# liuq-lab/bayesgm

Hardware: AMD Instinct MI355X
Metric: posterior samples/sec (whole node), CausalBGM N=1e6 p=200 (higher is better)
Workload: dtype f32

## Files before the change

### bayesgm_amd/csrc/bgm_host.h

```cpp
#pragma once
#include <hip/hip_runtime.h>

#include <algorithm>
#include <string>
#include <vector>

#include "../../include/bgm_hip.h"
#include "causal_kernels.h"
#include "fit_types.h"

void bgm_set_error(const std::string &msg);

#define BGM_HIP_CHECK(expr)                                                                  \
  do {                                                                                       \
    hipError_t _e = (expr);                                                                  \
    if (_e != hipSuccess) {                                                                  \
      bgm_set_error(std::string(#expr) + ": " + hipGetErrorString(_e));                      \
      return BGM_E_HIP;                                                                      \
    }                                                                                        \
  } while (0)

template <class T>
static int bgm_reserve(T *&ptr, size_t &cap, size_t count) {
  if (cap >= count) return BGM_OK;
// ... 44 lines not shown
};

struct bgm_handle {
  int device = 0;
  int n_cus = 256;
  int disc_norm = 0;
  bool configured = false;
  bgm_causal_config cfg{};
  int q = 0, p = 0;
  HostNet nets[4];
  CausalMeta meta{};
  int KT1 = 0, KSL1 = 0, NTL = 0;
  float *blob_dev = nullptr;
  size_t blob_cap = 0;
  bool blob_valid = false;
  float *sblob_dev = nullptr;
  size_t sblob_cap = 0;
  bool sblob_valid = false;
  float *gblob_dev = nullptr, *gram_w_dev = nullptr, *uc_dev = nullptr;
  size_t gblob_cap = 0, gram_w_cap = 0, uc_cap = 0;
  bool gram_valid = false;
  bool mh_direct = false;
  bool mh_all_ksteps = false;
  CausalMeta gmeta{};
  int precision = 0;
  unsigned char *bx_blob_dev = nullptr;
  size_t bx_cap = 0;
  float *eff_cache = nullptr;
  size_t eff_cache_cap = 0;
  int outcome_cache = 2;
  unsigned long long *eff_stats_dev = nullptr;
  unsigned long long eff_total = 0;
  unsigned long long ev_total = 0;
  float *ev_z = nullptr; unsigned *ev_meta = nullptr; int *ev_tile = nullptr, *ev_slot_cnt = nullptr; float *ev_out = nullptr, *ev_carry = nullptr;
  size_t ev_z_cap = 0, ev_meta_cap = 0, ev_tile_cap = 0, ev_slot_cap = 0, ev_out_cap = 0, ev_carry_cap = 0;
  int ev_carry_flip = 0;
  long long ev_budget_bytes = 0;
  int ev_fallbacks = 0;
  bool bx_valid = false;
  alignas(8) unsigned char bx_meta_store[192];
  const int32_t *prior_seg = nullptr;
  const float *prior_tab = nullptr;
  int prior_segments = 0;
  float *ra_scale = nullptr;
  const float *ra_up = nullptr, *ra_dn = nullptr;
  int ra_n = 0;
// ... 128 lines not shown
```

### bayesgm_amd/csrc/causal_api.hip

```cpp
#include <algorithm>
#include <string>
#include <vector>
#include <cstdio>
#include <cmath>
#include <cstring>
#include <cstdlib>

#include "causal_launch.h"
#include "bnf_det_host.h"
#include "gx_host.h"

static thread_local std::string g_err;
void bgm_set_error(const std::string &msg) { g_err = msg; }

extern "C" const char *bgm_last_error(void) { return g_err.c_str(); }
extern "C" const char *bgm_version(void) { return "bayesgm_amd-hip 0.1 (gfx950)"; }

extern "C" int bgm_create(bgm_handle **out, int device) {
  if (!out) { bgm_set_error("bgm_create: out == NULL"); return BGM_E_INVALID; }
  BGM_HIP_CHECK(hipSetDevice(device));
  hipDeviceProp_t prop;
  BGM_HIP_CHECK(hipGetDeviceProperties(&prop, device));
  if (std::string(prop.gcnArchName).find("gfx950") == std::string::npos) {
    bgm_set_error(std::string("bgm_create: device is ") + prop.gcnArchName + ", this library is built for gfx950 only");
    return BGM_E_UNSUPPORTED;
  }
  bgm_handle *h = new bgm_handle();
  h->device = device;
  h->n_cus = prop.multiProcessorCount;
  const char *direct = std::getenv("BGM_MH_DIRECT_LIKELIHOOD");
  h->mh_direct = direct != nullptr && std::strcmp(direct, "0") != 0;
  const char *all_ks = std::getenv("BGM_MH_ALL_KSTEPS");
  h->mh_all_ksteps = all_ks != nullptr && std::strcmp(all_ks, "0") != 0;
  *out = h;
  return BGM_OK;
}

extern "C" int bgm_set_disc_norm(bgm_handle *h, int32_t mode) {
  if (!h || (mode != 0 && mode != 1)) { bgm_set_error("bgm_set_disc_norm: mode must be 0 (batch statistics) or 1 (inference mode)"); return BGM_E_INVALID; }
  h->disc_norm = mode;
  return BGM_OK;
}

extern "C" int bgm_destroy(bgm_handle *h) {
  if (!h) return BGM_OK;
  hipSetDevice(h->device);
  if (h->blob_dev) hipFree(h->blob_dev);
  if (h->eblob_dev) hipFree(h->eblob_dev);
  if (h->sblob_dev) hipFree(h->sblob_dev);
  if (h->gblob_dev) hipFree(h->gblob_dev);
  if (h->gram_w_dev) hipFree(h->gram_w_dev);
  if (h->uc_dev) hipFree(h->uc_dev);
  if (h->bx_blob_dev) hipFree(h->bx_blob_dev);
  if (h->acc_scratch) hipFree(h->acc_scratch);
  if (h->eff_cache) hipFree(h->eff_cache);
  if (h->eff_stats_dev) hipFree(h->eff_stats_dev);
// ... 126 lines not shown
  const int q1 = q + 1;
  int KT1, KSL1, NTL;
  if (!bgm_causal_shape(q1, p + 1, KT1, KSL1, NTL)) {
    bgm_set_error("no compiled kernel shape contains this model (needs sum(z_dims) <= 19 and v_dim <= 207, or <= 159 when sum(z_dims) > 11)");
    return BGM_E_UNSUPPORTED;
  }
  h->KT1 = KT1; h->KSL1 = KSL1; h->NTL = NTL;
  CausalMeta &m = h->meta;
  std::memset(&m, 0, sizeof(m));
  m.q = q; m.p = p; m.binary = h->cfg.binary_treatment ? 1 : 0;
  m.sig_pc = p % 16; m.sig_slot = bgm_sig_slot(p, NTL);
  auto s2 = [](float s) { return s > 0.0f ? s * s : -1.0f; };
  m.sig2_v = s2(h->cfg.sigma_v); m.sig2_x = s2(h->cfg.sigma_x); m.sig2_y = s2(h->cfg.sigma_y);
  m.n_gh = h->cfg.n_hidden_g - 1;
  int off = 0;
  auto take = [&](int n) { int o = off; off += (n + 3) / 4 * 4; return o; };
  m.w1g = take(16 * KT1 * 64); m.w1f = take(16 * KT1 * 64); m.w1h = take(16 * KT1 * 64);
  m.b1g = take(64); m.b1f = take(64); m.b1h = take(64);
  m.wg = take(m.n_gh * 4096); m.bg = take(m.n_gh * 64);
  m.wgl = take(64 * 16 * NTL); m.bgl = take(16 * NTL);
  m.wf2 = take(64 * 32); m.bf2 = take(32); m.wf3 = take(32 * 16); m.bf3 = take(16); m.wf4 = take(16 * 16); m.bf4 = take(16);
  m.wh2 = take(64 * 32); m.bh2 = take(32); m.wh3 = take(32 * 16); m.bh3 = take(16); m.wh4 = take(16 * 16); m.bh4 = take(16);
  m.wxf = take(64);
  m.total = off;
  if ((size_t)m.total * 4 > 160 * 1024) {
    bgm_set_error("model does not fit the 160 KiB LDS-resident layout (" + std::to_string(m.total * 4) + " B); p <= 207 with default widths");
    return BGM_E_UNSUPPORTED;
  }
  blob.assign(m.total, 0.0f);
  auto ident = [](int rho) { return rho; };
  const L1RowMaps rm(h);
  pack_layer(blob, m.w1g, G.W(0), q, 64, KT1, 4, [&](int rho) { return rm.g(rho); });
  pack_layer(blob, m.w1f, F.W(0), z0 + z1 + 1, 64, KT1, 4, [&](int rho) { return rm.f(rho); });
  pack_layer(blob, m.w1h, H.W(0), z0 + z2, 64, KT1, 4, [&](int rho) { return rm.h(rho); });
  causal_l1_masks(h, KT1, KSL1, m.l1f, m.l1h, m.l1b);
  pack_bias(blob, m.b1g, G.b(0), 64, 4); pack_bias(blob, m.b1f, F.b(0), 64, 4); pack_bias(blob, m.b1h, H.b(0), 64, 4);
  for (int l = 0; l < m.n_gh; ++l) {
    pack_layer(blob, m.wg + l * 4096, G.W(1 + l), 64, 64, 4, 4, ident);
    pack_bias(blob, m.bg + l * 64, G.b(1 + l), 64, 4);
  }
  const int LG = (int)G.dims.size() - 2;
  {
    std::vector<float> Wp, bp;
    bgm_g_last_padded(G.W(LG), G.b(LG), p, NTL, Wp, bp);
    pack_layer(blob, m.wgl, Wp.data(), 64, 16 * NTL, 4, NTL, ident);
    pack_bias(blob, m.bgl, bp.data(), 16 * NTL, NTL);
  }
  pack_layer(blob, m.wf2, F.W(1), 64, 32, 4, 2, ident); pack_bias(blob, m.bf2, F.b(1), 32, 2);
  pack_layer(blob, m.wf3, F.W(2), 32, 8, 2, 1, ident); pack_bias(blob, m.bf3, F.b(2), 8, 1);
// ... 13 lines not shown
  const int w3[2] = {m.wf3, m.wh3}, b3[2] = {m.bf3, m.bh3}, w4[2] = {m.wf4, m.wh4}, b4[2] = {m.bf4, m.bh4};
#pragma unroll
  for (int k = 0; k < 2; ++k) {
    if (in(w3[k], 32 * 16)) {
      const int rho = (i - w3[k]) >> 4, f = tail_pos_to_feature((i - w3[k]) & 15);
      dst[i] = f >= 0 ? src[w3[k] + rho * 16 + f] * BGM_LRS_W : 0.0f;
      return;
    }
    if (in(b3[k], 16)) {
      const int f = tail_pos_to_feature(i - b3[k]);
      dst[i] = f >= 0 ? src[b3[k] + f] : 0.0f;
      return;
    }
    if (in(w4[k], 16 * 16)) {
      const int f = tail_pos_to_feature((i - w4[k]) >> 4), c = (i - w4[k]) & 3;
      dst[i] = (f >= 0 && c < 2) ? src[w4[k] + f * 16 + c] * BGM_LRS_W : 0.0f;
      return;
    }
    if (in(b4[k], 16)) {
      const int c = (i - b4[k]) & 3;
      dst[i] = c < 2 ? src[b4[k] + c] : 0.0f;
      return;
    }
  }
  const bool scaled = in(m.wg, m.n_gh * 4096) || in(m.wgl, 64 * 16 * NTL) || in(m.wf2, 64 * 32) || in(m.wh2, 64 * 32);
  dst[i] = scaled ? src[i] * BGM_LRS_W : src[i];
}

int bgm_causal_sampling_blob(bgm_handle *h, hipStream_t stream) {
  if (!h->blob_valid) h->sblob_valid = false;
  int rc = bgm_causal_build_blob(h, stream);
  if (rc) return rc;
  if (h->sblob_valid) return BGM_OK;
  const size_t n = (size_t)h->meta.total;
  if ((rc = bgm_reserve(h->sblob_dev, h->sblob_cap, n))) return rc;
  h->gram_valid = false;
  hipLaunchKernelGGL(causal_scale_blob_kernel, dim3((unsigned)((n + 255) / 256)), dim3(256), 0, stream, h->blob_dev, h->sblob_dev,
                     h->meta, h->NTL);
  BGM_HIP_CHECK(hipGetLastError());
  h->sblob_valid = true;
  return BGM_OK;
}

static bool gram_wanted(const bgm_handle *h, int NTL) { return !h->mh_direct && h->precision == 0 && NTL > 2; }

static float packed_w(const std::vector<float> &b, int off, int NT, int i, int o) {
// ... 21 lines not shown
    }
    act.swap(nxt);
  }
  std::vector<float> a0(64), W((size_t)64 * p), wt((size_t)65 * p), G(64 * 64);
  for (int i = 0; i < 64; ++i) a0[i] = (float)act[i];
  for (int i = 0; i < 64; ++i)
    for (int c = 0; c < p; ++c) W[(size_t)i * p + c] = packed_w(sb, m.wgl, NTL, i, c);
  for (int c = 0; c < p; ++c) {
    double s = sb[m.bgl + c];
    for (int i = 0; i < 64; ++i) { s += (double)W[(size_t)i * p + c] * (double)a0[i]; wt[(size_t)c * 64 + i] = W[(size_t)i * p + c]; }
    wt[(size_t)64 * p + c] = (float)s;
  }
  for (int i = 0; i < 64; ++i)
    for (int k = 0; k <= i; ++k) {
      double s = 0.0;
      for (int c = 0; c < p; ++c) s += (double)W[(size_t)i * p + c] * (double)W[(size_t)k * p + c];
      G[i * 64 + k] = G[k * 64 + i] = (float)s;
    }
  CausalMeta gm = m;
  gm.bgl = m.wgl + 4096;
  const int shift = (gm.bgl + 132) - m.wf2;
  for (int CausalMeta::*f : {&CausalMeta::wf2, &CausalMeta::bf2, &CausalMeta::wf3, &CausalMeta::bf3, &CausalMeta::wf4, &CausalMeta::bf4,
                             &CausalMeta::wh2, &CausalMeta::bh2, &CausalMeta::wh3, &CausalMeta::bh3, &CausalMeta::wh4, &CausalMeta::bh4,
                             &CausalMeta::wxf, &CausalMeta::total})
    gm.*f += shift;
  std::vector<float> gb((size_t)gm.total, 0.0f);
  std::copy(sb.begin(), sb.begin() + m.wgl, gb.begin());
  pack_layer(gb, gm.wgl, G.data(), 64, 64, 4, 4, [](int rho) { return rho; });
  for (int i = 0; i < 64; ++i) { gb[gm.bgl + i] = a0[i]; gb[gm.bgl + 64 + i] = packed_w(sb, m.wgl, NTL, i, m.sig_slot); }
  gb[gm.bgl + 128] = sb[m.bgl + m.sig_slot];
  std::copy(sb.begin() + m.wf2, sb.end(), gb.begin() + gm.wf2);
  if (int rc = bgm_reserve(h->gblob_dev, h->gblob_cap, gb.size())) return rc;
  if (int rc = bgm_reserve(h->gram_w_dev, h->gram_w_cap, wt.size())) return rc;
  BGM_HIP_CHECK(hipMemcpyAsync(h->gblob_dev, gb.data(), gb.size() * sizeof(float), hipMemcpyHostToDevice, stream));
  BGM_HIP_CHECK(hipMemcpyAsync(h->gram_w_dev, wt.data(), wt.size() * sizeof(float), hipMemcpyHostToDevice, stream));
  BGM_HIP_CHECK(hipStreamSynchronize(stream));
  h->gmeta = gm;
  h->gram_valid = true;
  h->hmc_valid = false;
  return BGM_OK;
}

static __global__ __launch_bounds__(256) void causal_gram_prepass_kernel(const float *wt, const float *v, long long n, int p, float *uc) {
  extern __shared__ __attribute__((aligned(16))) float sw[];
  for (int i = threadIdx.x; i < 65 * p; i += blockDim.x) sw[i] = wt[i];
  __syncthreads();
  const long long row = (long long)blockIdx.x * blockDim.x + threadIdx.x;
// ... 72 lines not shown
  if (gx_wanted(h)) {
    return gx_logpost(h, x, y, v, z, n, out, stream);
  }
  if (bnf_det_wanted(h)) {
    if (h->prior_seg || h->precision != 0) { bgm_set_error("bgm_causal_logpost: the conditional prior / split precision exist for the LDS-resident shapes only"); return BGM_E_UNSUPPORTED; }
    return bnf_det_logpost(h, x, y, v, z, n, out, stream);
  }
  int rc = bgm_causal_sampling_blob(h, stream);
  if (rc) return rc;
  const int grid = mh_grid(h, n);
  if (h->precision != 0) return bgm_causal_bx3_logpost(h, x, y, v, z, n, out, grid, stream);
  if (h->prior_seg) return bgm_causal_prior_logpost(h, x, y, v, z, n, out, grid, stream);
  return bgm_causal_dispatch(h, "kernel", [&](auto s) {
    using S = decltype(s);
    return bgm_launch(causal_logpost_kernel<S::KT1, S::KSL1, S::NTL, MH_R, MH_WAVES>, grid, MH_WAVES, h->meta.total * 4, stream,
                      h->sblob_dev, h->meta, x, y, v, z, n, out, nullptr, nullptr);
  });
}

template <int EFFECT>
static int launch_mh(bgm_handle *h, const CausalMhKArgs &ka, int grid, int lds, hipStream_t stream) {
  return bgm_causal_dispatch(h, "MH kernel", [&](auto s) {
    using S = decltype(s);
    return bgm_launch(ka.uc ? causal_mh_kernel<S::KT1, S::KSL1, S::NTL, MH_R, MH_WAVES, EFFECT, 0, (S::NTL > 2)>
                            : causal_mh_kernel<S::KT1, S::KSL1, S::NTL, MH_R, MH_WAVES, EFFECT>,
                      grid, MH_WAVES, lds, stream, ka);
  });
}

extern "C" int bgm_causal_mh_run(bgm_handle *h, const bgm_mh_args *a, void *stream_) {
  if (!h || !h->configured) { bgm_set_error("bgm_causal_mh_run: handle not configured"); return BGM_E_STATE; }
  if (!a) { bgm_set_error("bgm_causal_mh_run: NULL args"); return BGM_E_INVALID; }
  if (a->n <= 0 || a->n_iters <= 0) return BGM_OK;
  if (!a->x_dev || !a->y_dev || !a->v_dev || !a->state_dev || !a->logp_dev) { bgm_set_error("bgm_causal_mh_run: NULL data pointer"); return BGM_E_INVALID; }
  if (a->row_base + a->n > 0xFFFFFFFFll) { bgm_set_error("bgm_causal_mh_run: row index exceeds the 32-bit RNG counter"); return BGM_E_INVALID; }
  if (a->effect == BGM_EFFECT_ADRF && (!a->x_values_dev || a->n_doses <= 0 || !a->adrf_partial_dev)) { bgm_set_error("bgm_causal_mh_run: ADRF effect needs x_values / adrf_partial"); return BGM_E_INVALID; }
  if (a->effect == BGM_EFFECT_ITE && !a->ite_dev) { bgm_set_error("bgm_causal_mh_run: ITE effect needs ite_dev"); return BGM_E_INVALID; }
  if (a->effect == BGM_EFFECT_ADRF && h->cfg.binary_treatment) { bgm_set_error("bgm_causal_mh_run: ADRF effect on a binary-treatment model"); return BGM_E_INVALID; }
  const int it_end = a->it_begin + a->n_iters;
  if ((a->effect != BGM_EFFECT_NONE || a->draws_dev) && it_end - a->burn_in > a->n_keep) { bgm_set_error("bgm_causal_mh_run: iterations beyond burn_in + n_keep"); return BGM_E_INVALID; }
  hipStream_t stream = (hipStream_t)stream_;
  BGM_HIP_CHECK(hipSetDevice(h->device));
  if (h->ra_scale) {
    const char *path = gx_wanted(h) ? "the general-width engine (hidden widths outside the compiled families)"
                       : bnf_det_wanted(h) ? "the streamed-fragment kernels (no LDS-resident compiled shape holds the model)"
                       : h->precision != 0 ? "the split-precision kernels (bgm_causal_set_precision)"
                       : h->prior_seg ? "the conditional latent prior (bgm_causal_set_prior)" : nullptr;
    if (path) { bgm_set_error(std::string("bgm_causal_mh_run: the per-chain proposal scale (bgm_causal_set_row_scale) does not exist for ") + path); return BGM_E_UNSUPPORTED; }
  }
// ... 271 lines not shown
```

### bayesgm_amd/csrc/causal_event_api.hip

```cpp
#include <algorithm>
#include <cstdlib>
#include <string>

#include "causal_launch.h"
#include "causal_event_kernels.h"

static constexpr int EV_SPREAD_WAVES = 4, EV_SPREAD_LDS_FLOATS = 8192;

bool bgm_causal_event_wanted(const bgm_handle *h, int effect, int n_doses) {
  static const bool off = std::getenv("BGM_NO_EVENT_SPLIT") != nullptr;
  if (off || h->outcome_cache != 2) return false;
  if (effect == BGM_EFFECT_ITE) return h->cfg.binary_treatment != 0;
  return effect == BGM_EFFECT_ADRF && n_doses >= 1 && (n_doses + 3) / 4 <= EV_NCMAX;
}

template <class T>
static int ev_try_reserve(T *&ptr, size_t &cap, size_t need) {
  if (cap >= need) return BGM_OK;
  if (ptr) BGM_HIP_CHECK(hipFree(ptr));
  ptr = nullptr; cap = 0;
  if (hipMalloc((void **)&ptr, need * sizeof(T)) != hipSuccess) {
    (void)hipGetLastError();
    ptr = nullptr;
    return 1;
// ... 46 lines not shown
  h->ev_z_cap = h->ev_meta_cap = h->ev_tile_cap = h->ev_slot_cap = h->ev_out_cap = h->ev_carry_cap = 0;
}

int bgm_causal_event_mh_launch(bgm_handle *h, CausalMhKArgs &ka, int grid, int lds, hipStream_t stream) {
  ka.ev_z = h->ev_z; ka.ev_meta = h->ev_meta; ka.tile_ev = h->ev_tile; ka.slot_cnt = h->ev_slot_cnt;
  if (h->precision != 0) return bgm_causal_bx3_mh_launch(h, ka, 3, grid, stream);
  if (h->prior_seg) return bgm_causal_prior_mh_launch(h, ka, 3, grid, lds, stream);
  if (ka.row_scale) return bgm_causal_rowadapt_mh_launch(h, ka, 3, grid, lds, stream);
  return bgm_causal_dispatch(h, "event-form MH kernel", [&](auto s) {
    using S = decltype(s);
    return bgm_launch(ka.uc ? causal_mh_kernel<S::KT1, S::KSL1, S::NTL, MH_R, MH_WAVES, 3, 0, (S::NTL > 2)>
                            : causal_mh_kernel<S::KT1, S::KSL1, S::NTL, MH_R, MH_WAVES, 3>,
                      grid, MH_WAVES, lds, stream, ka);
  });
}

int bgm_causal_event_finish(bgm_handle *h, const CausalMhKArgs &ka, int grid, int first, hipStream_t stream, int effect) {
  CausalEventFArgs fa{};
  fa.blob = ka.blob; fa.ev_z = h->ev_z; fa.slot_cnt = h->ev_slot_cnt; fa.ev_cap = ka.ev_cap; fa.n_doses = ka.n_doses;
  fa.x_values = ka.x_values; fa.ev_out = reinterpret_cast<float2 *>(h->ev_out); fa.eff_stats = ka.eff_stats; fa.m = ka.m;
  constexpr int FW = 4, WPS = 2;
  const int rc = bgm_causal_dispatch(h, "event-form outcome-net kernel", [&](auto s) {
    using S = decltype(s);
    const int lds = 4 * (16 * S::KT1 * 64 + 64 + 64 * 32 + 32 + 32 * 16 + 16 + 16 * 16 + 16 + 64);
    return bgm_launch(effect == BGM_EFFECT_ITE ? causal_event_f_ite_kernel<S::KT1, S::KSL1, FW, WPS>
                                               : causal_event_f_kernel<S::KT1, S::KSL1, FW, WPS>,
                      grid * MH_WAVES * WPS / FW, FW, lds, stream, fa);
  });
  if (rc) return rc;
  if (effect == BGM_EFFECT_ITE) {
    CausalEventIteArgs ia{};
    ia.n = ka.n; ia.row_base = ka.row_base; ia.it_begin = ka.it_begin; ia.n_iters = ka.n_iters; ia.burn_in = ka.burn_in; ia.n_keep = ka.n_keep;
    ia.sample_y = ka.sample_y; ia.n_slots = grid * MH_WAVES; ia.k0 = ka.k0; ia.k1 = ka.k1;
    ia.ev_meta = h->ev_meta; ia.tile_ev = h->ev_tile; ia.ev_cap = ka.ev_cap; ia.ev_out = reinterpret_cast<const float4 *>(h->ev_out);
    const size_t carry_floats = (size_t)((ka.n + 15) / 16) * 64 * 2;
    h->ev_carry_flip = first ? 0 : (h->ev_carry_flip ^ 1);
    ia.carry_in = reinterpret_cast<const float4 *>(h->ev_carry + (h->ev_carry_flip ^ 1) * carry_floats);
    ia.carry_out = reinterpret_cast<float4 *>(h->ev_carry + h->ev_carry_flip * carry_floats);
    ia.first = first; ia.ite = ka.ite;
    hipLaunchKernelGGL(causal_event_ite_kernel, dim3((unsigned)((ka.n + 255) / 256)), dim3(256), 0, stream, ia);
    BGM_HIP_CHECK(hipGetLastError());
    return BGM_OK;
  }
  CausalEventSpreadArgs sa{};
  sa.n = ka.n; sa.row_base = ka.row_base; sa.it_begin = ka.it_begin; sa.n_iters = ka.n_iters; sa.burn_in = ka.burn_in; sa.n_keep = ka.n_keep;
  sa.sample_y = ka.sample_y; sa.n_doses = ka.n_doses; sa.k0 = ka.k0; sa.k1 = ka.k1;
  sa.ev_meta = h->ev_meta; sa.tile_ev = h->ev_tile; sa.ev_cap = ka.ev_cap; sa.ev_out = reinterpret_cast<const float2 *>(h->ev_out);
  const size_t carry_floats = (size_t)((ka.n + 15) / 16) * (size_t)((ka.n_doses + 3) / 4) * 64 * 2;
  h->ev_carry_flip = first ? 0 : (h->ev_carry_flip ^ 1);
// ... 15 lines not shown
```

### bayesgm_amd/csrc/causal_event_kernels.h

```cpp
#pragma once
#include "causal_kernels.h"

#define EV_NCMAX 8

struct CausalEventFArgs {
  const float *blob;
  const float *ev_z;
  const int *slot_cnt;
  long long ev_cap;
  int n_doses;
  const float *x_values;
  float2 *ev_out;
  unsigned long long *eff_stats;
  CausalMeta m;
};

template <int KT1, int KSL1, int WAVES, int WPS>
__global__ __launch_bounds__(64 * WAVES) void causal_event_f_kernel(CausalEventFArgs a) {
  extern __shared__ __attribute__((aligned(16))) float lds[];
  CausalMeta m = a.m;
  {
    int off = 0;
    auto put = [&](int src, int nfl) {
      for (int i = threadIdx.x; i < nfl; i += 64 * WAVES) lds[off + i] = a.blob[src + i];
      const int o = off;
      off += nfl;
      return o;
    };
    m.w1f = put(a.m.w1f, 16 * KT1 * 64); m.b1f = put(a.m.b1f, 64);
    m.wf2 = put(a.m.wf2, 64 * 32); m.bf2 = put(a.m.bf2, 32); m.wf3 = put(a.m.wf3, 32 * 16); m.bf3 = put(a.m.bf3, 16);
    m.wf4 = put(a.m.wf4, 16 * 16); m.bf4 = put(a.m.bf4, 16); m.wxf = put(a.m.wxf, 64);
    __syncthreads();
  }
  const int lane = threadIdx.x & 63, wave = threadIdx.x >> 6;
  const int j = lane & 15, g = lane >> 4, lane_off = 64 * g + j;
  const long long wid = (long long)blockIdx.x * WAVES + wave;
  const long long slot = wid / WPS;
  const int sub = (int)(wid % WPS);
  const int cnt = a.slot_cnt[slot];
  const int n_calls = (a.n_doses + 3) >> 2;
  if (a.eff_stats != nullptr && lane == 0 && sub == 0 && cnt > 0) atomicAdd(&a.eff_stats[1], (unsigned long long)cnt);
  for (int e0 = 16 * sub; e0 < cnt; e0 += 16 * WPS) {
    BGM_NO_HOIST();
    const int el = (e0 + j < cnt) ? e0 + j : cnt - 1;
    const float *zr = a.ev_z + (slot * a.ev_cap + el) * (long long)m.q;
    f32x4 zs[1][KT1];
#pragma unroll
    for (int t = 0; t < KT1; ++t)
#pragma unroll
      for (int r = 0; r < 4; ++r) {
        const int f = 16 * t + 4 * r + g;
        zs[0][t][r] = (f < m.q) ? zr[f] : 0.0f;
      }
    const unsigned rowid[1] = {0u};
    const bool valid[1] = {true};
    float2 *out = a.ev_out + ((slot * a.ev_cap + e0) >> 4) * (long long)n_calls * 64;
    causal_effects<KT1, KSL1, 1, 1, true, true, true>(lds, m, lane_off, g, j, lane, zs, rowid, valid, 0ll, 16ll, 0u, 0ll, 1, 0, a.n_doses,
                                                      a.x_values, nullptr, nullptr, 0u, 0u, out);
  }
}

template <int KT1, int KSL1, int WAVES, int WPS>
__global__ __launch_bounds__(64 * WAVES) void causal_event_f_ite_kernel(CausalEventFArgs a) {
  extern __shared__ __attribute__((aligned(16))) float lds[];
  CausalMeta m = a.m;
  {
    int off = 0;
    auto put = [&](int src, int nfl) {
      for (int i = threadIdx.x; i < nfl; i += 64 * WAVES) lds[off + i] = a.blob[src + i];
      const int o = off;
      off += nfl;
      return o;
    };
    m.w1f = put(a.m.w1f, 16 * KT1 * 64); m.b1f = put(a.m.b1f, 64);
    m.wf2 = put(a.m.wf2, 64 * 32); m.bf2 = put(a.m.bf2, 32); m.wf3 = put(a.m.wf3, 32 * 16); m.bf3 = put(a.m.bf3, 16);
    m.wf4 = put(a.m.wf4, 16 * 16); m.bf4 = put(a.m.bf4, 16); m.wxf = put(a.m.wxf, 64);
    __syncthreads();
  }
  const int lane = threadIdx.x & 63, wave = threadIdx.x >> 6;
  const int j = lane & 15, g = lane >> 4, lane_off = 64 * g + j;
  const long long wid = (long long)blockIdx.x * WAVES + wave;
// ... 183 lines not shown
```

### bayesgm_amd/csrc/causal_kernels.h

```cpp
#pragma once
#include "bgm_device.h"
#include "row_tails.h"

struct CausalMeta {
  int q, p;
  int sig_pc, sig_slot;
  int binary;
  float sig2_v, sig2_x, sig2_y;
  int n_gh;
  int w1g, w1f, w1h, b1g, b1f, b1h;
  int wg, bg;
  int wgl, bgl;
  int wf2, bf2, wf3, bf3, wf4, bf4;
  int wh2, bh2, wh3, bh3, wh4, bh4;
  int wxf;
  int total;
  unsigned l1f, l1h, l1b;
};
__host__ __device__ constexpr bool causal_l1_masked(int KT1, int PRIOR) { return !(PRIOR != 0 && KT1 > 1); }

struct CausalMhKArgs {
  const float *blob;
  const float *x, *y, *v;
  const float *uc;
  long long n, row_base;
  float *state, *logp;
  int init, it_begin, n_iters, burn_in;
  float q_sd;
  unsigned k0, k1;
  unsigned *acc_count;
  float *draws;
  int n_keep, sample_y, n_doses;
  const float *x_values;
  float *adrf_partial;
  float *ite;
  unsigned long long *clk;
  const int *seg;
  const float *prior_tab;
  float *eff_cache;
  int eff_skip;
  unsigned long long *eff_stats;
  float *ev_z;
// ... 425 lines not shown
    unsigned long long tsec[8] = {0, 0, 0, 0, 0, 0, 0, 0}, tlast = 0;
    causal_logp<KT1, KSL1, NTL, R>(lds, m, lane_off, g, j, zin, vreg, xr, yr, lp, tsec, tlast);
#else
    causal_logp<KT1, KSL1, NTL, R>(lds, m, lane_off, g, j, zin, vreg, xr, yr, lp);
#endif
    if constexpr (PRIOR) {
      PriorRow<KT1> pr;
      const long long rowc = (row0 + j < n) ? row0 + j : n - 1;
      pr.load(seg, prior_tab, rowc, m.q, g);
      lp[0] += pr.correction(zin[0], m.q, g);
    }
#pragma unroll
    for (int rr = 0; rr < R; ++rr) {
      const long long row = row0 + 16 * rr + j;
      if (g == 0 && row < n) out[row] = lp[rr];
    }
  }
}

__device__ __forceinline__ float pick_by_group(int g, float v0, float v1, float v2, float v3) {
  return g == 0 ? v0 : (g == 1 ? v1 : (g == 2 ? v2 : v3));
}

template <int KT1, int KSL1, int R, int EFFECT, bool GROUPING = true, bool CACHE = false, bool EVAL_ONLY = false, bool L1MASK = true,
          bool ROWS = false, bool TAILS = false>
__device__ __forceinline__ void causal_effects(const float *lds, const CausalMeta &m, int lane_off, int g, int j,
                                               int lane, const f32x4 (&zs)[R][KT1], const unsigned (&rowid)[R],
                                               const bool (&valid)[R], long long row0, long long n, unsigned it,
                                               long long d, int n_keep, int sample_y, int n_doses,
                                               const float *x_values, float *adrf_slot, float *ite, unsigned k0,
                                               unsigned k1, float2 *cache = nullptr, float *ite_c = nullptr,
                                               float *row_mom = nullptr, float *row_y = nullptr, int label = 0,
                                               float *row_tails = nullptr, int k_tail = 0) {
  static_assert(!ROWS || (EFFECT == 1 && R == 1 && GROUPING && !CACHE && !EVAL_ONLY), "ROWS: the grouped finish of the dose-response sums");
  static_assert(EFFECT != 4 || (R == 1 && !CACHE && !EVAL_ONLY && !ROWS), "EFFECT 4: the label sums of one row tile per wave");
  static_assert(!TAILS || ROWS, "TAILS: the tail buffers of the per-row dose-response");
  constexpr bool ARMS = (EFFECT == 2 || EFFECT == 4);
  BGM_NO_HOIST();
  f32x4 z0in[R][KT1];
#pragma unroll
  for (int rr = 0; rr < R; ++rr)
#pragma unroll
    for (int t = 0; t < KT1; ++t)
#pragma unroll
      for (int r = 0; r < 4; ++r) z0in[rr][t][r] = (16 * t + 4 * r + g == m.q) ? 0.0f : zs[rr][t][r];
  f32x4 base[R][4];
  if constexpr (L1MASK) dense_masked<KT1, KSL1, 4, R>(lds + m.w1f, lds + m.b1f, lane_off, g, z0in, base, m.l1b);
  else dense<KT1, KSL1, 4, R>(lds + m.w1f, lds + m.b1f, lane_off, g, z0in, base);
  f32x4 wx[4];
#pragma unroll
  for (int t = 0; t < 4; ++t) wx[t] = *reinterpret_cast<const f32x4 *>(lds + m.wxf + 16 * t + 4 * g);
  const int nd = ARMS ? (CACHE && n_doses == 0 ? 0 : 2) : n_doses;
  constexpr int DB = ARMS ? 2 : 4;
  constexpr bool GROUPED = (EFFECT == 1 && R == 1 && GROUPING);
  const int n_calls = (nd + 3) >> 2, n_own = GROUPED ? (n_calls & ~3) : 0;
  f32x4 nz[R];
#pragma unroll
  for (int rr = 0; rr < R; ++rr) nz[rr] = f32x4{0.0f, 0.0f, 0.0f, 0.0f};
  for (int kb = 0; kb < n_calls; ++kb) {
    BGM_NO_HOIST();
    const bool own = kb < n_own;
    const int c4 = kb & ~3, p4 = kb & 3;
    if (!EVAL_ONLY && sample_y && (!own || p4 == 0)) {
#pragma unroll
      for (int rr = 0; rr < R; ++rr) nz[rr] = box_muller4(philox4x32_10(rowid[rr], it, (unsigned)(own ? c4 + g : kb), TAG_YNOISE, k0, k1));
    }
    float xk[DB];
#pragma unroll
    for (int e = 0; e < DB; ++e) {
      const int k = own ? 4 * (c4 + e) + p4 : 4 * kb + e;
      xk[e] = ARMS ? (e == 0 ? 1.0f : 0.0f) : x_values[k < nd ? k : nd - 1];
    }
    float mu[DB * R], sr[DB * R];
#ifndef BGM_NO_JIT_EFFECTS
    if constexpr (R == 1) {
      f32x4 a2[DB][2];
#pragma unroll
// ... 170 lines not shown
  if (g == 0 && row < n) ite[row * (long long)n_keep + d] = y1 - y0;
}

template <int KT1>
__device__ __forceinline__ void causal_event_append(const CausalMhKArgs &a, int q, long long slot, int &ev_cnt, bool ev, int g, int j,
                                                    const f32x4 (&z)[KT1], int it) {
  const unsigned m16 = (unsigned)(__ballot(ev && g == 0) & 0xFFFFull);
  if (m16 == 0u) return;
  if (ev) {
    const long long e = slot * a.ev_cap + ev_cnt + __popc(m16 & ((1u << j) - 1u));
    float *ez = a.ev_z + e * (long long)q;
#pragma unroll
    for (int t = 0; t < KT1; ++t)
#pragma unroll
      for (int r = 0; r < 4; ++r) {
        const int f = 16 * t + 4 * r + g;
        if (f < q) ez[f] = z[t][r];
      }
    if (g == 0) a.ev_meta[e] = ((unsigned)(it - a.it_begin) << 4) | (unsigned)j;
  }
  ev_cnt += __popc(m16);
}

template <int KT1, int KSL1, int NTL, int R, int WAVES, int EFFECT, int PRIOR = 0, bool GRAM = false, bool ROWADAPT = false>
__global__ __launch_bounds__(64 * WAVES) void causal_mh_kernel(CausalMhKArgs a) {
  static_assert(PRIOR == 0 || R == 1, "conditional prior: one row tile per wave");
  constexpr bool L1M = causal_l1_masked(KT1, PRIOR);
  extern __shared__ __attribute__((aligned(16))) float lds[];
  const CausalMeta &m = a.m;
  lds_fill(lds, a.blob, m.total);
  const int lane = threadIdx.x & 63, wave = threadIdx.x >> 6;
  const int j = lane & 15, g = lane >> 4, lane_off = 64 * g + j;
  const long long n = a.n;
  const long long n_tiles = (n + 16 * R - 1) / (16 * R);
  const long long slot = (long long)blockIdx.x * WAVES + wave;
  const long long n_slots = (long long)gridDim.x * WAVES;
  const unsigned long long clk_c0 = __builtin_readcyclecounter(), clk_r0 = __builtin_amdgcn_s_memrealtime();
#ifdef BGM_PROF
  unsigned long long tsec[8] = {0, 0, 0, 0, 0, 0, 0, 0}, tlast = 0;
#endif
  const int wave_u = __builtin_amdgcn_readfirstlane(wave);
  volatile __attribute__((address_space(3))) int *prog =
      (volatile __attribute__((address_space(3))) int *)((__attribute__((address_space(3))) float *)lds + m.total);
  if (lane == 0) prog[wave_u] = 0;
  int tiles_done = 0;
  [[maybe_unused]] int ev_cnt = 0;

  for (long long tile = slot; tile < n_tiles; tile += n_slots) {
    const long long row0 = tile * 16 * R;
// ... 126 lines not shown
        if (a.draws != nullptr) {
#pragma unroll
          for (int rr = 0; rr < R; ++rr) {
            const long long row = row0 + 16 * rr + j;
            if (row < n) {
              float *dr = a.draws + (d * n + row) * (long long)m.q;
#pragma unroll
              for (int t = 0; t < KT1; ++t)
#pragma unroll
                for (int r = 0; r < 4; ++r) {
                  const int f = 16 * t + 4 * r + g;
                  if (f < m.q) dr[f] = zs[rr][t][r];
                }
            }
          }
        }
        if constexpr (EFFECT == 3) {
          static_assert(R == 1, "event mode: one row tile per wave");
          causal_event_append<KT1>(a, m.q, slot, ev_cnt, valid[0] && (moved[0] || (a.ev_first && it == a.it_begin)), g, j, zs[0], it);
        } else if constexpr (EFFECT == 1 && R == 1) {
          float2 *cache = reinterpret_cast<float2 *>(a.eff_cache) + slot * (long long)((a.n_doses + 3) >> 2) * 64;
          float *adrf_slot = a.adrf_partial + slot * (long long)a.n_doses * a.n_keep;
          const bool skip = a.eff_skip && eff_cached && accmask == 0ull;
          causal_effects<KT1, KSL1, R, EFFECT, true, true, false, L1M>(lds, m, lane_off, g, j, lane, zs, rowid, valid, row0, n, (unsigned)it, d, a.n_keep,
                                                            a.sample_y, skip ? 0 : a.n_doses, a.x_values, adrf_slot, a.ite, a.k0, a.k1, cache);
          if (skip) causal_effects_cached(g, j, lane, rowid[0], valid[0], (unsigned)it, d, a.sample_y, a.n_doses, adrf_slot, a.k0, a.k1, cache);
          eff_cached = true;
          n_eff_skipped += skip ? 1u : 0u;
        } else if constexpr (EFFECT == 2 && R == 1) {
          const bool skip = a.eff_skip && eff_cached && accmask == 0ull;
          causal_effects<KT1, KSL1, R, EFFECT, true, true, false, L1M>(lds, m, lane_off, g, j, lane, zs, rowid, valid, row0, n, (unsigned)it, d, a.n_keep,
                                                            a.sample_y, skip ? 0 : 2, a.x_values, a.adrf_partial, a.ite, a.k0, a.k1, nullptr, ite_c);
          if (skip) causal_ite_cached(g, j, rowid[0], row0 + j, n, (unsigned)it, d, a.n_keep, a.sample_y, a.ite, a.k0, a.k1, ite_c);
          eff_cached = true;
          n_eff_skipped += skip ? 1u : 0u;
        } else if constexpr (EFFECT != 0) {
          causal_effects<KT1, KSL1, R, EFFECT, true, false, false, L1M>(lds, m, lane_off, g, j, lane, zs, rowid, valid, row0, n, (unsigned)it, d,
                                                a.n_keep, a.sample_y, a.n_doses, a.x_values,
                                                a.adrf_partial + slot * (long long)((EFFECT == 2) ? 2 : a.n_doses) * a.n_keep,
                                                a.ite, a.k0, a.k1);
        }
      }
    }
    if constexpr (EFFECT != 0 && R == 1) {
      if (a.eff_stats != nullptr && lane == 0 && n_eff_skipped != 0u) atomicAdd(&a.eff_stats[0], (unsigned long long)n_eff_skipped);
    }
    if constexpr (EFFECT == 3) {
// ... 171 lines not shown
```

### bayesgm_amd/csrc/causal_launch.h

```cpp
#pragma once
#include <algorithm>
#include <string>
#include <type_traits>

#include "bgm_host.h"

#ifndef BGM_MH_R
#define BGM_MH_R 1
#endif
#ifndef BGM_MH_WAVES
#define BGM_MH_WAVES 8
#endif
static constexpr int MH_R = BGM_MH_R, MH_WAVES = BGM_MH_WAVES;
static_assert(MH_R == 1, "BGM_MH_R != 1: the conditional-prior, per-chain-scale, event-form and split-precision MH kernels exist for one row "
                         "tile per wave only, and they share the grid and the per-slot buffers of the default path");

static inline int bgm_causal_grid(const bgm_handle *h, int64_t n, int row_tiles) {
  return bgm_tile_grid(h, (n + 16 * row_tiles - 1) / (16 * row_tiles), MH_WAVES);
}

template <int KT1_, int KSL1_, int NTL_>
struct CausalShape { static constexpr int KT1 = KT1_, KSL1 = KSL1_, NTL = NTL_; };
template <class... S>
struct CausalShapeList {};
// ... 14 lines not shown
}
static_assert(bgm_causal_shapes_cover(), "bgm_causal_shape() returns a (KT1, KSL1, NTL) that is not in CausalShapes");

template <class F, class... S>
static int bgm_causal_dispatch(CausalShapeList<S...>, int KT1, int KSL1, int NTL, const char *what, F &&f) {
  int rc = BGM_E_UNSUPPORTED;
  if (!(... || (S::KT1 == KT1 && S::KSL1 == KSL1 && S::NTL == NTL && ((rc = f(S{})), true))))
    bgm_set_error(std::string("no compiled ") + what + " variant for (KT1,KSL1,NTL)=(" + std::to_string(KT1) + "," + std::to_string(KSL1) + "," +
                  std::to_string(NTL) + ")");
  return rc;
}
template <class F>
static int bgm_causal_dispatch(const bgm_handle *h, const char *what, F &&f) {
  return bgm_causal_dispatch(CausalShapes{}, h->KT1, h->KSL1, h->NTL, what, f);
}

template <class F>
static int bgm_causal_with_effect(int effect, F &&f) {
  if (effect == 3) return f(std::integral_constant<int, 3>{});
  if (effect == BGM_EFFECT_ADRF) return f(std::integral_constant<int, 1>{});
  if (effect == BGM_EFFECT_ITE) return f(std::integral_constant<int, 2>{});
  return f(std::integral_constant<int, 0>{});
}
```

### bayesgm_amd/csrc/causal_rowadapt_api.hip

```cpp
#include <cmath>
#include <string>

#include "causal_launch.h"

extern "C" int bgm_causal_set_row_scale(bgm_handle *h, float *scale_dev, const float *up_dev, const float *dn_dev, int32_t n_table,
                                        float s_min, float s_max) {
  if (!h) { bgm_set_error("bgm_causal_set_row_scale: NULL handle"); return BGM_E_INVALID; }
  if (!scale_dev) {
    h->ra_scale = nullptr; h->ra_up = h->ra_dn = nullptr; h->ra_n = 0; h->ra_min = h->ra_max = 0.0f;
    return BGM_OK;
  }
  if (n_table < 0 || (n_table > 0 && (!up_dev || !dn_dev))) { bgm_set_error("bgm_causal_set_row_scale: up_dev / dn_dev must hold n_table >= 0 factors"); return BGM_E_INVALID; }
  if (!(s_min > 0.0f) || !(s_max >= s_min) || !std::isfinite(s_max)) { bgm_set_error("bgm_causal_set_row_scale: the clamp needs 0 < s_min <= s_max < inf"); return BGM_E_INVALID; }
  h->ra_scale = scale_dev; h->ra_up = up_dev; h->ra_dn = dn_dev; h->ra_n = n_table; h->ra_min = s_min; h->ra_max = s_max;
  return BGM_OK;
}

int bgm_causal_rowadapt_mh_launch(bgm_handle *h, const CausalMhKArgs &ka, int effect, int grid, int lds, hipStream_t stream) {
  if (!ka.row_scale || ka.seg) { bgm_set_error("per-chain proposal scale: launched without a scale buffer / with a conditional prior"); return BGM_E_STATE; }
  return bgm_causal_with_effect(effect, [&](auto e) {
    return bgm_causal_dispatch(h, "per-chain proposal scale: MH kernel", [&](auto s) {
      using S = decltype(s);
      constexpr int EFFECT = decltype(e)::value;
      return bgm_launch(ka.uc ? causal_mh_kernel<S::KT1, S::KSL1, S::NTL, MH_R, MH_WAVES, EFFECT, 0, (S::NTL > 2), true>
                              : causal_mh_kernel<S::KT1, S::KSL1, S::NTL, MH_R, MH_WAVES, EFFECT, 0, false, true>,
                        grid, MH_WAVES, lds, stream, ka);
    });
  });
}
```

Measured before the change: 1.283 billion.

## Compute outcome-net tail layers on vector ALU interleaved with next dose's MFMA layer

Adds a vector-ALU implementation of the outcome network's last two layers for the grouped dose-response path. It stores a repacked LDS copy of those weights, and the tail of one dose batch is interleaved step by step with the MFMA layer-2 of the next batch. The aim is to keep matrix and vector units busy at the same time instead of running small, poorly shaped MFMA tails serially. In exchange it uses more LDS and registers, adds permlane reductions, and creates more kernel variants. It is gated by shape rules and an environment flag that restores the MFMA tails.

```diff
diff --git a/bayesgm_amd/csrc/bgm_host.h b/bayesgm_amd/csrc/bgm_host.h
--- a/bayesgm_amd/csrc/bgm_host.h
+++ b/bayesgm_amd/csrc/bgm_host.h
@@ -90,6 +90,7 @@
   bool gram_valid = false;
   bool mh_direct = false;
   bool mh_all_ksteps = false;
+  bool mh_mfma_tails = false;
   CausalMeta gmeta{};
   int precision = 0;
   unsigned char *bx_blob_dev = nullptr;
diff --git a/bayesgm_amd/csrc/causal_api.hip b/bayesgm_amd/csrc/causal_api.hip
--- a/bayesgm_amd/csrc/causal_api.hip
+++ b/bayesgm_amd/csrc/causal_api.hip
@@ -32,6 +32,8 @@
   h->mh_direct = direct != nullptr && std::strcmp(direct, "0") != 0;
   const char *all_ks = std::getenv("BGM_MH_ALL_KSTEPS");
   h->mh_all_ksteps = all_ks != nullptr && std::strcmp(all_ks, "0") != 0;
+  const char *mfma_tails = std::getenv("BGM_MH_MFMA_TAILS");
+  h->mh_mfma_tails = mfma_tails != nullptr && std::strcmp(mfma_tails, "0") != 0;
   *out = h;
   return BGM_OK;
 }
@@ -204,9 +206,12 @@
   m.wf2 = take(64 * 32); m.bf2 = take(32); m.wf3 = take(32 * 16); m.bf3 = take(16); m.wf4 = take(16 * 16); m.bf4 = take(16);
   m.wh2 = take(64 * 32); m.bh2 = take(32); m.wh3 = take(32 * 16); m.bh3 = take(16); m.wh4 = take(16 * 16); m.bh4 = take(16);
   m.wxf = take(64);
+  const int layers = off;
+  m.vf3 = take(4 * 8 * 8); m.vf4 = take(8 * 2 + 8 + 2);
   m.total = off;
   if ((size_t)m.total * 4 > 160 * 1024) {
-    bgm_set_error("model does not fit the 160 KiB LDS-resident layout (" + std::to_string(m.total * 4) + " B); p <= 207 with default widths");
+    const std::string copy = (size_t)layers * 4 <= 160 * 1024 ? " beside the " + std::to_string((m.total - layers) * 4) + " B vector-ALU copy of f's tail" : "";
+    bgm_set_error("model does not fit the 160 KiB LDS-resident layout (" + std::to_string(layers * 4) + " B)" + copy + "; p <= 207 with default widths");
     return BGM_E_UNSUPPORTED;
   }
   blob.assign(m.total, 0.0f);
@@ -266,6 +271,16 @@
       dst[i] = c < 2 ? src[b4[k] + c] : 0.0f;
       return;
     }
+  }
+  if (in(m.vf3, 256)) {
+    const int e = i - m.vf3, g = e >> 6, l = (e >> 3) & 7, o = e & 7;
+    dst[i] = src[m.wf3 + (16 * (l >> 2) + 4 * g + (l & 3)) * 16 + o] * BGM_LRS_W;
+    return;
+  }
+  if (in(m.vf4, 28)) {
+    const int e = i - m.vf4;
+    dst[i] = e < 16 ? src[m.wf4 + (e >> 1) * 16 + (e & 1)] * BGM_LRS_W : e < 24 ? src[m.bf3 + e - 16] : e < 26 ? src[m.bf4 + e - 24] : 0.0f;
+    return;
   }
   const bool scaled = in(m.wg, m.n_gh * 4096) || in(m.wgl, 64 * 16 * NTL) || in(m.wf2, 64 * 32) || in(m.wh2, 64 * 32);
   dst[i] = scaled ? src[i] * BGM_LRS_W : src[i];
@@ -333,7 +348,7 @@
   const int shift = (gm.bgl + 132) - m.wf2;
   for (int CausalMeta::*f : {&CausalMeta::wf2, &CausalMeta::bf2, &CausalMeta::wf3, &CausalMeta::bf3, &CausalMeta::wf4, &CausalMeta::bf4,
                              &CausalMeta::wh2, &CausalMeta::bh2, &CausalMeta::wh3, &CausalMeta::bh3, &CausalMeta::wh4, &CausalMeta::bh4,
-                             &CausalMeta::wxf, &CausalMeta::total})
+                             &CausalMeta::wxf, &CausalMeta::vf3, &CausalMeta::vf4, &CausalMeta::total})
     gm.*f += shift;
   std::vector<float> gb((size_t)gm.total, 0.0f);
   std::copy(sb.begin(), sb.begin() + m.wgl, gb.begin());
@@ -452,9 +467,13 @@
 static int launch_mh(bgm_handle *h, const CausalMhKArgs &ka, int grid, int lds, hipStream_t stream) {
   return bgm_causal_dispatch(h, "MH kernel", [&](auto s) {
     using S = decltype(s);
-    return bgm_launch(ka.uc ? causal_mh_kernel<S::KT1, S::KSL1, S::NTL, MH_R, MH_WAVES, EFFECT, 0, (S::NTL > 2)>
-                            : causal_mh_kernel<S::KT1, S::KSL1, S::NTL, MH_R, MH_WAVES, EFFECT>,
-                      grid, MH_WAVES, lds, stream, ka);
+    return bgm_causal_with_tails(EFFECT == 1 && !h->mh_mfma_tails, [&](auto vt) {
+      constexpr bool VT = EFFECT == 1 && decltype(vt)::value;
+      constexpr bool VT_G = VT && causal_valu_tails(S::KT1, S::NTL, S::NTL > 2), VT_D = VT && causal_valu_tails(S::KT1, S::NTL, false);
+      return bgm_launch(ka.uc ? causal_mh_kernel<S::KT1, S::KSL1, S::NTL, MH_R, MH_WAVES, EFFECT, 0, (S::NTL > 2), false, VT_G>
+                              : causal_mh_kernel<S::KT1, S::KSL1, S::NTL, MH_R, MH_WAVES, EFFECT, 0, false, false, VT_D>,
+                        grid, MH_WAVES, lds, stream, ka);
+    });
   });
 }
 
diff --git a/bayesgm_amd/csrc/causal_event_api.hip b/bayesgm_amd/csrc/causal_event_api.hip
--- a/bayesgm_amd/csrc/causal_event_api.hip
+++ b/bayesgm_amd/csrc/causal_event_api.hip
@@ -92,9 +92,10 @@
   constexpr int FW = 4, WPS = 2;
   const int rc = bgm_causal_dispatch(h, "event-form outcome-net kernel", [&](auto s) {
     using S = decltype(s);
-    const int lds = 4 * (16 * S::KT1 * 64 + 64 + 64 * 32 + 32 + 32 * 16 + 16 + 16 * 16 + 16 + 64);
+    const bool vt = effect != BGM_EFFECT_ITE && !h->mh_mfma_tails && !h->prior_seg && causal_valu_tails(S::KT1, S::NTL, ka.uc != nullptr, ka.row_scale != nullptr);
+    const int lds = 4 * (16 * S::KT1 * 64 + 64 + 64 * 32 + 32 + 32 * 16 + 16 + 16 * 16 + 16 + 64 + (vt ? 256 + 28 : 0));
     return bgm_launch(effect == BGM_EFFECT_ITE ? causal_event_f_ite_kernel<S::KT1, S::KSL1, FW, WPS>
-                                               : causal_event_f_kernel<S::KT1, S::KSL1, FW, WPS>,
+                      : vt ? causal_event_f_kernel<S::KT1, S::KSL1, FW, WPS, true> : causal_event_f_kernel<S::KT1, S::KSL1, FW, WPS>,
                       grid * MH_WAVES * WPS / FW, FW, lds, stream, fa);
   });
   if (rc) return rc;
diff --git a/bayesgm_amd/csrc/causal_event_kernels.h b/bayesgm_amd/csrc/causal_event_kernels.h
--- a/bayesgm_amd/csrc/causal_event_kernels.h
+++ b/bayesgm_amd/csrc/causal_event_kernels.h
@@ -15,7 +15,7 @@
   CausalMeta m;
 };
 
-template <int KT1, int KSL1, int WAVES, int WPS>
+template <int KT1, int KSL1, int WAVES, int WPS, bool VTAILS = false>
 __global__ __launch_bounds__(64 * WAVES) void causal_event_f_kernel(CausalEventFArgs a) {
   extern __shared__ __attribute__((aligned(16))) float lds[];
   CausalMeta m = a.m;
@@ -30,6 +30,7 @@
     m.w1f = put(a.m.w1f, 16 * KT1 * 64); m.b1f = put(a.m.b1f, 64);
     m.wf2 = put(a.m.wf2, 64 * 32); m.bf2 = put(a.m.bf2, 32); m.wf3 = put(a.m.wf3, 32 * 16); m.bf3 = put(a.m.bf3, 16);
     m.wf4 = put(a.m.wf4, 16 * 16); m.bf4 = put(a.m.bf4, 16); m.wxf = put(a.m.wxf, 64);
+    if constexpr (VTAILS) { m.vf3 = put(a.m.vf3, 256); m.vf4 = put(a.m.vf4, 28); }
     __syncthreads();
   }
   const int lane = threadIdx.x & 63, wave = threadIdx.x >> 6;
@@ -55,8 +56,8 @@
     const unsigned rowid[1] = {0u};
     const bool valid[1] = {true};
     float2 *out = a.ev_out + ((slot * a.ev_cap + e0) >> 4) * (long long)n_calls * 64;
-    causal_effects<KT1, KSL1, 1, 1, true, true, true>(lds, m, lane_off, g, j, lane, zs, rowid, valid, 0ll, 16ll, 0u, 0ll, 1, 0, a.n_doses,
-                                                      a.x_values, nullptr, nullptr, 0u, 0u, out);
+    causal_effects<KT1, KSL1, 1, 1, true, true, true, true, false, false, VTAILS>(lds, m, lane_off, g, j, lane, zs, rowid, valid, 0ll, 16ll, 0u, 0ll, 1,
+                                                                                  0, a.n_doses, a.x_values, nullptr, nullptr, 0u, 0u, out);
   }
 }
 
diff --git a/bayesgm_amd/csrc/causal_kernels.h b/bayesgm_amd/csrc/causal_kernels.h
--- a/bayesgm_amd/csrc/causal_kernels.h
+++ b/bayesgm_amd/csrc/causal_kernels.h
@@ -1,4 +1,7 @@
 #pragma once
+#include <type_traits>
+#include <utility>
+
 #include "bgm_device.h"
 #include "row_tails.h"
 
@@ -14,10 +17,16 @@
   int wf2, bf2, wf3, bf3, wf4, bf4;
   int wh2, bh2, wh3, bh3, wh4, bh4;
   int wxf;
+  int vf3;
+  int vf4;
   int total;
   unsigned l1f, l1h, l1b;
 };
 __host__ __device__ constexpr bool causal_l1_masked(int KT1, int PRIOR) { return !(PRIOR != 0 && KT1 > 1); }
+
+__host__ __device__ constexpr bool causal_valu_tails(int KT1, int NTL, bool GRAM, bool ROWADAPT = false) {
+  return !(KT1 > 1 && GRAM) && !(NTL == 7 && !GRAM) && !(ROWADAPT && KT1 > 1 && NTL == 2);
+}
 
 struct CausalMhKArgs {
   const float *blob;
@@ -489,8 +498,166 @@
   return g == 0 ? v0 : (g == 1 ? v1 : (g == 2 ? v2 : v3));
 }
 
+template <int... S, class F>
+__device__ __forceinline__ void vt_static_for(std::integer_sequence<int, S...>, F &&f) { (f(std::integral_constant<int, S>{}), ...); }
+
+struct VtTail {
+  float act[4][8];
+  float p[4][8];
+  float mu, sr, tot;
+  int k;
+  bool own;
+};
+
+__device__ __forceinline__ float vt_swap32_add(float v0, float v1) {
+  const auto s = __builtin_amdgcn_permlane32_swap(__builtin_bit_cast(unsigned, v0), __builtin_bit_cast(unsigned, v1), false, false);
+  return __builtin_bit_cast(float, (unsigned)s[0]) + __builtin_bit_cast(float, (unsigned)s[1]);
+}
+__device__ __forceinline__ float vt_swap16_add(float v0, float v1) {
+  const auto s = __builtin_amdgcn_permlane16_swap(__builtin_bit_cast(unsigned, v0), __builtin_bit_cast(unsigned, v1), false, false);
+  return __builtin_bit_cast(float, (unsigned)s[0]) + __builtin_bit_cast(float, (unsigned)s[1]);
+}
+
+template <int S, bool CACHE, bool EVAL_ONLY>
+__device__ __forceinline__ void vt_tail_step(VtTail &T, const float *w3v, const float *w4v, int lane, int pass, float sig2_y, int sample_y,
+                                             bool valid, int nd, f32x4 &nz, int g, float2 *cache) {
+  if constexpr (S <= 10) {
+#pragma unroll
+    for (int grp = 3 * S; grp < (3 * S + 3 < 32 ? 3 * S + 3 : 32); ++grp) {
+      const int l = grp >> 2, e = grp & 3;
+      const f32x4 wa = *reinterpret_cast<const f32x4 *>(w3v + 8 * l), wb = *reinterpret_cast<const f32x4 *>(w3v + 8 * l + 4);
+      const float a = T.act[e][l];
+#pragma unroll
+      for (int o = 0; o < 8; ++o) {
+        const float w = o < 4 ? wa[o & 3] : wb[o & 3];
+        T.p[e][o] = l == 0 ? w * a : fmaf(w, a, T.p[e][o]);
+      }
+    }
+  } else if constexpr (S == 11) {
+#pragma unroll
+    for (int o = 0; o < 8; ++o) {
+      T.p[0][o] = vt_swap32_add(T.p[0][o], T.p[2][o]);
+      T.p[1][o] = vt_swap32_add(T.p[1][o], T.p[3][o]);
+    }
+  } else if constexpr (S == 12) {
+    const f32x4 ba = *reinterpret_cast<const f32x4 *>(w4v + 16), bb = *reinterpret_cast<const f32x4 *>(w4v + 20);
+#pragma unroll
+    for (int o = 0; o < 8; ++o) T.p[0][o] = vt_swap16_add(T.p[0][o], T.p[1][o]) + (o < 4 ? ba[o & 3] : bb[o & 3]);
+  } else if constexpr (S == 13) {
+    const f32x4 b4 = *reinterpret_cast<const f32x4 *>(w4v + 24);
+    float mu = b4[0], sr = b4[1];
+#pragma unroll
+    for (int o4 = 0; o4 < 4; ++o4) {
+      const f32x4 w = *reinterpret_cast<const f32x4 *>(w4v + 4 * o4);
+#pragma unroll
+      for (int h = 0; h < 2; ++h) {
+        const float a = lrelu_s(T.p[0][2 * o4 + h]);
+        mu = fmaf(w[2 * h], a, mu);
+        sr = fmaf(w[2 * h + 1], a, sr);
+      }
+    }
+    T.mu = mu; T.sr = sr;
+  } else if constexpr (S == 14) {
+    const float s2 = (sig2_y > 0.0f) ? sig2_y : softplus_f(T.sr) + BGM_EPS;
+    const float sd_m = __builtin_sqrtf(s2);
+    if constexpr (CACHE) cache[pass * 64 + lane] = make_float2(T.mu, sd_m);
+    if constexpr (EVAL_ONLY) return;
+    const float noise = T.own ? nz[0] : pick_by_group(g, nz[0], nz[1], nz[2], nz[3]);
+    if (T.own) nz = f32x4{nz[1], nz[2], nz[3], nz[0]};
+    const float y = sample_y ? fmaf(sd_m, noise, T.mu) : T.mu;
+    T.tot = (valid && T.k < nd) ? y : 0.0f;
+  } else if constexpr (!EVAL_ONLY) {
+    T.tot = sum_over_j_to_lane15(T.tot);
+  }
+}
+
+template <class F>
+__device__ __forceinline__ void vt_layer2(const float *lds, const CausalMeta &m, int lane_off, int g, const f32x4 (&base)[4],
+                                          const f32x4 (&wx)[4], const float (&xk)[4], f32x4 (&a2)[4][2], F &&fill) {
+#pragma unroll
+  for (int u = 0; u < 2; ++u) {
+    const f32x4 b = *reinterpret_cast<const f32x4 *>(lds + m.bf2 + 16 * u + 4 * g);
+#pragma unroll
+    for (int e = 0; e < 4; ++e) a2[e][u] = b;
+  }
+  const float *w2 = lds + m.wf2 + lane_off * 2;
+  vt_static_for(std::make_integer_sequence<int, 16>{}, [&](auto S) {
+    constexpr int s = decltype(S)::value, t = s >> 2, r = s & 3;
+    AFrag<2> af;
+    af.load(w2 + (16 * t + r) * 16 * 2);
+    float bop[4];
+#pragma unroll
+    for (int e = 0; e < 4; ++e) bop[e] = lrelu_s_pinned(fmaf(wx[t][r], xk[e], base[t][r]));
+#pragma unroll
+    for (int u = 0; u < 2; ++u)
+#pragma unroll
+      for (int e = 0; e < 4; ++e) a2[e][u] = BGM_MFMA(af.get(u), bop[e], a2[e][u]);
+    fill(S);
+  });
+}
+
+template <bool CACHE, bool EVAL_ONLY>
+__device__ __forceinline__ void causal_dose_passes_valu(const float *lds, const CausalMeta &m, int lane_off, int g, int j, int lane,
+                                                        const f32x4 (&base)[4], const f32x4 (&wx)[4], unsigned rowid, bool valid,
+                                                        unsigned it, long long d, int sample_y, int nd, const float *x_values,
+                                                        float *adrf_slot, unsigned k0, unsigned k1, float2 *cache) {
+  const int n_calls = (nd + 3) >> 2, n_own = n_calls & ~3;
+  if (n_calls == 0) return;
+  const float *w3v = lds + m.vf3 + 64 * g, *w4v = lds + m.vf4;
+  f32x4 nz = f32x4{0.0f, 0.0f, 0.0f, 0.0f};
+  f32x4 a2[4][2];
+  VtTail T;
+  auto doses = [&](int kb, float (&xk)[4]) {
+    const bool own = kb < n_own;
+#pragma unroll
+    for (int e = 0; e < 4; ++e) {
+      const int k = own ? 4 * ((kb & ~3) + e) + (kb & 3) : 4 * kb + e;
+      xk[e] = x_values[k < nd ? k : nd - 1];
+    }
+  };
+  auto noise = [&](int kb) {
+    const bool own = kb < n_own;
+    if (!EVAL_ONLY && sample_y && (!own || (kb & 3) == 0)) nz = box_muller4(philox4x32_10(rowid, it, (unsigned)(own ? (kb & ~3) + g : kb), TAG_YNOISE, k0, k1));
+  };
+  auto open_tail = [&](int pass) {
+    T.own = pass < n_own;
+    T.k = T.own ? 4 * ((pass & ~3) + g) + (pass & 3) : 4 * pass + g;
+#pragma unroll
+    for (int e = 0; e < 4; ++e)
+#pragma unroll
+      for (int l = 0; l < 8; ++l) T.act[e][l] = lrelu_s(a2[e][l >> 2][l & 3]);
+  };
+  auto emit = [&]() {
+    if constexpr (EVAL_ONLY) return;
+    if (j == 15 && T.k < nd) unsafeAtomicAdd(adrf_slot + (long long)d * nd + T.k, T.tot);
+  };
+  {
+    float xk[4];
+    doses(0, xk);
+    vt_layer2(lds, m, lane_off, g, base, wx, xk, a2, [](auto) {});
+    noise(0);
+  }
+  for (int kb = 1; kb < n_calls; ++kb) {
+    BGM_NO_HOIST();
+    float xk[4];
+    doses(kb, xk);
+    open_tail(kb - 1);
+    vt_layer2(lds, m, lane_off, g, base, wx, xk, a2, [&](auto S) {
+      vt_tail_step<decltype(S)::value, CACHE, EVAL_ONLY>(T, w3v, w4v, lane, kb - 1, m.sig2_y, sample_y, valid, nd, nz, g, cache);
+    });
+    emit();
+    noise(kb);
+  }
+  BGM_NO_HOIST();
+  open_tail(n_calls - 1);
+  vt_static_for(std::make_integer_sequence<int, 16>{}, [&](auto S) {
+    vt_tail_step<decltype(S)::value, CACHE, EVAL_ONLY>(T, w3v, w4v, lane, n_calls - 1, m.sig2_y, sample_y, valid, nd, nz, g, cache);
+  });
+  emit();
+}
+
 template <int KT1, int KSL1, int R, int EFFECT, bool GROUPING = true, bool CACHE = false, bool EVAL_ONLY = false, bool L1MASK = true,
-          bool ROWS = false, bool TAILS = false>
+          bool ROWS = false, bool TAILS = false, bool VTAILS = false>
 __device__ __forceinline__ void causal_effects(const float *lds, const CausalMeta &m, int lane_off, int g, int j,
                                                int lane, const f32x4 (&zs)[R][KT1], const unsigned (&rowid)[R],
                                                const bool (&valid)[R], long long row0, long long n, unsigned it,
@@ -520,6 +687,12 @@
   const int nd = ARMS ? (CACHE && n_doses == 0 ? 0 : 2) : n_doses;
   constexpr int DB = ARMS ? 2 : 4;
   constexpr bool GROUPED = (EFFECT == 1 && R == 1 && GROUPING);
+  if constexpr (VTAILS) {
+    static_assert(GROUPED && !ROWS && (CACHE || !EVAL_ONLY), "VTAILS: the grouped dose-response sums of the MH kernels and of their event form");
+    causal_dose_passes_valu<CACHE, EVAL_ONLY>(lds, m, lane_off, g, j, lane, base[0], wx, rowid[0], valid[0], it, d, sample_y, nd, x_values, adrf_slot,
+                                   k0, k1, cache);
+    return;
+  }
   const int n_calls = (nd + 3) >> 2, n_own = GROUPED ? (n_calls & ~3) : 0;
   f32x4 nz[R];
 #pragma unroll
@@ -736,9 +909,10 @@
   ev_cnt += __popc(m16);
 }
 
-template <int KT1, int KSL1, int NTL, int R, int WAVES, int EFFECT, int PRIOR = 0, bool GRAM = false, bool ROWADAPT = false>
+template <int KT1, int KSL1, int NTL, int R, int WAVES, int EFFECT, int PRIOR = 0, bool GRAM = false, bool ROWADAPT = false, bool VTAILS = false>
 __global__ __launch_bounds__(64 * WAVES) void causal_mh_kernel(CausalMhKArgs a) {
   static_assert(PRIOR == 0 || R == 1, "conditional prior: one row tile per wave");
+  static_assert(!VTAILS || (EFFECT == 1 && R == 1), "VTAILS: the grouped dose-response sums");
   constexpr bool L1M = causal_l1_masked(KT1, PRIOR);
   extern __shared__ __attribute__((aligned(16))) float lds[];
   const CausalMeta &m = a.m;
@@ -911,7 +1085,7 @@
           float2 *cache = reinterpret_cast<float2 *>(a.eff_cache) + slot * (long long)((a.n_doses + 3) >> 2) * 64;
           float *adrf_slot = a.adrf_partial + slot * (long long)a.n_doses * a.n_keep;
           const bool skip = a.eff_skip && eff_cached && accmask == 0ull;
-          causal_effects<KT1, KSL1, R, EFFECT, true, true, false, L1M>(lds, m, lane_off, g, j, lane, zs, rowid, valid, row0, n, (unsigned)it, d, a.n_keep,
+          causal_effects<KT1, KSL1, R, EFFECT, true, true, false, L1M, false, false, VTAILS>(lds, m, lane_off, g, j, lane, zs, rowid, valid, row0, n, (unsigned)it, d, a.n_keep,
                                                             a.sample_y, skip ? 0 : a.n_doses, a.x_values, adrf_slot, a.ite, a.k0, a.k1, cache);
           if (skip) causal_effects_cached(g, j, lane, rowid[0], valid[0], (unsigned)it, d, a.sample_y, a.n_doses, adrf_slot, a.k0, a.k1, cache);
           eff_cached = true;
diff --git a/bayesgm_amd/csrc/causal_launch.h b/bayesgm_amd/csrc/causal_launch.h
--- a/bayesgm_amd/csrc/causal_launch.h
+++ b/bayesgm_amd/csrc/causal_launch.h
@@ -60,3 +60,8 @@
   if (effect == BGM_EFFECT_ITE) return f(std::integral_constant<int, 2>{});
   return f(std::integral_constant<int, 0>{});
 }
+
+template <class F>
+static int bgm_causal_with_tails(bool valu, F &&f) {
+  return valu ? f(std::true_type{}) : f(std::false_type{});
+}
diff --git a/bayesgm_amd/csrc/causal_rowadapt_api.hip b/bayesgm_amd/csrc/causal_rowadapt_api.hip
--- a/bayesgm_amd/csrc/causal_rowadapt_api.hip
+++ b/bayesgm_amd/csrc/causal_rowadapt_api.hip
@@ -22,9 +22,13 @@
     return bgm_causal_dispatch(h, "per-chain proposal scale: MH kernel", [&](auto s) {
       using S = decltype(s);
       constexpr int EFFECT = decltype(e)::value;
-      return bgm_launch(ka.uc ? causal_mh_kernel<S::KT1, S::KSL1, S::NTL, MH_R, MH_WAVES, EFFECT, 0, (S::NTL > 2), true>
-                              : causal_mh_kernel<S::KT1, S::KSL1, S::NTL, MH_R, MH_WAVES, EFFECT, 0, false, true>,
-                        grid, MH_WAVES, lds, stream, ka);
+      return bgm_causal_with_tails(EFFECT == 1 && !h->mh_mfma_tails, [&](auto vt) {
+        constexpr bool VT = EFFECT == 1 && decltype(vt)::value;
+        constexpr bool VT_G = VT && causal_valu_tails(S::KT1, S::NTL, S::NTL > 2, true), VT_D = VT && causal_valu_tails(S::KT1, S::NTL, false, true);
+        return bgm_launch(ka.uc ? causal_mh_kernel<S::KT1, S::KSL1, S::NTL, MH_R, MH_WAVES, EFFECT, 0, (S::NTL > 2), true, VT_G>
+                                : causal_mh_kernel<S::KT1, S::KSL1, S::NTL, MH_R, MH_WAVES, EFFECT, 0, false, true, VT_D>,
+                          grid, MH_WAVES, lds, stream, ka);
+      });
     });
   });
 }
```

New measurement: 1.328 billion (median of 6 runs). 1.04x the previous value.
